# harrisonvanderbyl/rwkv-cpp-accelerated

Hardware: AMD Instinct MI355X
Metric: tokens/sec single-stream RWKV-4 uint8 greedy decode (higher is better)
Workload: dtype u8 weights x 23-bit fixed-point activations, exact 32-bit integer accumulate (tile form: v_mfma_i32_16x16x64_i8 on signed limbs; row form: v_dot4_u32_u8 on the VALU); f32/f64 epilogues, f64 state; 1 GPU; RWKV-4-Raven-7B uint8 single-stream greedy decode (L=32, D=4096, V=50277), 32-token prompt then 1885-token continuation, device-resident state; parallelism=1 GPU

## Files before the change

rwkv-cpp-accelerated_amd/csrc/kernels.hip.h:

```cpp
#pragma once
#include <hip/hip_runtime.h>
#include <stdint.h>

namespace rwkvk {

constexpr int NT = 512;
constexpr int NW = NT / 64;
constexpr int RED_BYTES = 1024;
#define RWKV_ARGS_NOW(...) asm volatile("" ::RWKV_ARGS_S(__VA_ARGS__))
#define RWKV_ARGS_S(...) RWKV_ARGS_PICK(__VA_ARGS__, RWKV_A8, RWKV_A7, RWKV_A6, RWKV_A5, RWKV_A4, RWKV_A3, RWKV_A2, RWKV_A1)(__VA_ARGS__)
#define RWKV_ARGS_PICK(a, b, c, d, e, f, g, h, N, ...) N
#define RWKV_A1(a) "s"(a)
#define RWKV_A2(a, ...) "s"(a), RWKV_A1(__VA_ARGS__)
#define RWKV_A3(a, ...) "s"(a), RWKV_A2(__VA_ARGS__)
#define RWKV_A4(a, ...) "s"(a), RWKV_A3(__VA_ARGS__)
#define RWKV_A5(a, ...) "s"(a), RWKV_A4(__VA_ARGS__)
#define RWKV_A6(a, ...) "s"(a), RWKV_A5(__VA_ARGS__)
#define RWKV_A7(a, ...) "s"(a), RWKV_A6(__VA_ARGS__)
#define RWKV_A8(a, ...) "s"(a), RWKV_A7(__VA_ARGS__)
__device__ __forceinline__ int wave_id() { return __builtin_amdgcn_readfirstlane((int)(threadIdx.x >> 6)); }
__device__ __forceinline__ int block_lo(int n) { return (int)(((unsigned)blockIdx.x * (unsigned)n) / gridDim.x); }
__device__ __forceinline__ int block_hi(int n) { return (int)((((unsigned)blockIdx.x + 1u) * (unsigned)n) / gridDim.x); }
constexpr unsigned VOCAB = 50277u;
constexpr float QLIM = 4194000.0f;
// ... 554 lines not shown
        {
            float *redf = reinterpret_cast<float *>(red + RED_MAX);
            const double ws = wave_sum(ps);
            const float wm = wave_max(pm);
            if (lane == 0) { red[RED_OFFS + wave] = ws; redf[wave] = wm; }
            tl_stamp(tl, 3);
            if (SPLIT) {
                if (lane == 0) __hip_atomic_fetch_add(spin, 1u, __ATOMIC_RELEASE, __HIP_MEMORY_SCOPE_WORKGROUP);
                while (__hip_atomic_load(spin, __ATOMIC_ACQUIRE, __HIP_MEMORY_SCOPE_WORKGROUP) < (unsigned)NWP) __builtin_amdgcn_s_sleep(1);
            } else {
                __syncthreads();
            }
            double ts = 0.0; float tm = 0.f;
#pragma unroll
            for (int i = 0; i < NWP; i++) { ts += red[RED_OFFS + i]; tm = fmaxf(tm, redf[i]); }
            Sf = (float)ts; amax = tm;
        }
        tl_stamp(tl, 4);
#pragma unroll
        for (int q = 0; q < NVEC; q++)
#pragma unroll
            for (int i = 0; i < NQP; i++) {
                const int qd = threadIdx.x + i * NTP;
                if (qd < S * 256) stage_quad(xq + q * XVD, qd, vl[q][i], inv_scale(amax), qd < nqd);
            }
        if (SPLIT && threadIdx.x == 0) { bc[0] = Sf; bc[4] = amax; }
        __syncthreads();
        group_load<R, S, SPLIT ? 0 : pre_steps<S>(), S>(w, wb, stride, chunks, lane);
    }
    if (SPLIT) { Sf = bc[0]; amax = bc[4]; }
    tl_stamp(tl, 5);
}

constexpr size_t CU_LDS_BYTES = 160 * 1024;
__host__ __device__ constexpr int row_nvec(int cls) { return cls == 1 ? 3 : cls == 3 ? 2 : cls == 4 ? 4 : 1; }
struct RowLds { size_t red = 0, xq = 0, bval = 0, bidx = 0, bytes = 0; };
__host__ __device__ constexpr RowLds row_lds_of(int cls, int S)
{
    RowLds l;
    l.xq = l.red + RED_BYTES;
    l.bval = l.xq + (size_t)row_nvec(cls) * S * xvd<1>() * 4;
    l.bidx = l.bval + (cls == 5 ? NW * sizeof(float) : 0);
    l.bytes = l.bidx + (cls == 5 ? NW * sizeof(unsigned) : 0);
    return l;
}
template <int CLS, int S> struct RowGeo {
    static constexpr RowLds L = row_lds_of(CLS, S);
    static_assert(L.xq % 16 == 0 && L.bval == L.xq + (size_t)row_nvec(CLS) * xvd<S>() * 4, "the staged vectors: 16-byte pieces, xvd<S>() words each");
    static_assert(row_lds_of(CLS, 5).bytes <= CU_LDS_BYTES, "LDS layout at S = 5");
};

__device__ __forceinline__ unsigned lds_addr(const void *p)
{
    return (unsigned)(unsigned long long)(const __attribute__((address_space(3))) void *)p;
}
__device__ __forceinline__ void dma_piece_shared(const uint8_t *src, unsigned lds_dst)
{
    unsigned keep;
    asm volatile("s_mov_b32 %0, m0\n\ts_mov_b32 m0, %2\n\ts_nop 0\n\tglobal_load_lds_dwordx4 %1, off\n\ts_mov_b32 m0, %0"
                 : "=&s"(keep) : "v"(src), "s"(lds_dst) : "memory");
}
__device__ __forceinline__ void loader_clean_slate() { __builtin_amdgcn_s_waitcnt(0x0F70); }
template <int N> __device__ __forceinline__ void wait_vm() { asm volatile("s_waitcnt vmcnt(%0)" ::"n"(N) : "memory"); }
constexpr int GLDS_SPIN = 1 << 18;
__device__ __forceinline__ void wait_count(const unsigned *p, unsigned least, unsigned &fail)
{
    bool ok = false;
    for (int it = 0; it < GLDS_SPIN; it++) {
        if (__hip_atomic_load(p, __ATOMIC_ACQUIRE, __HIP_MEMORY_SCOPE_WORKGROUP) >= least) { ok = true; break; }
        __builtin_amdgcn_s_sleep(1);
    }
    fail = ok ? fail : 3u;
}
__device__ __forceinline__ void ring_report(unsigned fail, unsigned *herr)
{
    if (fail != 0u && herr != nullptr && (threadIdx.x & 63) == 0) __hip_atomic_store(herr, fail, __ATOMIC_RELAXED, __HIP_MEMORY_SCOPE_SYSTEM);
}
#ifndef RWKV_RING_DEPTH
#define RWKV_RING_DEPTH 28
#endif
#ifndef RWKV_RING_PRE
#define RWKV_RING_PRE 8
#endif
#ifndef RWKV_TEST_DROP_GROUP
#define RWKV_TEST_DROP_GROUP 0
#endif
#ifndef RWKV_RING_PRE_DEPTH
#define RWKV_RING_PRE_DEPTH 20
#endif
constexpr int NC = NW - 1;

struct FirstArgs {
    const float *embed;
    const double *ln;
    double *x;
    const double *x_in;
    SiteStatic st;
    SiteDyn dy;
    const double *sxy;
    size_t slot_stride;
    const Ctl *ctl;
    int D;
    int from_token;
};
__global__ __launch_bounds__(NT) void k_first(FirstArgs a)
{
    __shared__ double red[RED_BYTES / 8];
    const int D = a.D;
    const int j0 = block_lo(D), j1 = block_hi(D);
    const size_t so = (size_t)a.ctl->slot * a.slot_stride;
    double mean = 0.0, rstd = 1.0;
    const float *row = a.from_token ? a.embed + (size_t)a.ctl->token * D : nullptr;
    if (a.from_token) {
        double s[2] = {0.0, 0.0};
        for (int j = threadIdx.x; j < D; j += NT) { const double v = (double)row[j]; s[0] += v; s[1] += v * v; }
        block_sum<2>(s, red + RED_STATS);
        mean = s[0] / (double)D;
        rstd = 1.0 / sqrt((s[1] - s[0] * mean) / (double)(D - 1));
        __syncthreads();
    }
    SiteAcc<3> acc;
    acc.clear();
    for (int j = j0 + threadIdx.x; j < j1; j += NT) {
        double x;
        if (a.from_token) { x = a.ln[j] * (((double)row[j] - mean) * rstd) + a.ln[D + j]; a.x[j] = x; }
        else { x = a.x_in[j]; a.x[j] = x; }
        SitePre<3> pre;
        site_prefetch<3>(a.st, j, pre);
        site_emit<3>(pre, a.dy, D, j, x, a.sxy[so + j], acc);
    }
    site_publish<3, 64>(acc, a.dy, red);
}

struct AttArgs {
    const double *x;
    SiteStatic st;
    SiteDyn dy;
    const uint8_t *w;
    const unsigned *rs;
    const double *uw, *ew;
    const float *r_att, *o_att;
    double *saa, *sbb;
    size_t slot_stride;
    float *ybuf;
    double *partS;
    float *partM;
    const Ctl *ctl;
    int D;
    int ns;
    unsigned long long *tl;
    unsigned *herr;
};

__device__ __forceinline__ void att_epilogue(double *saa, double *sbb, float *ybuf, int g, double aa, double bb, double e1, double ek, float v, float r, double ew, float ra, float oa, double &part, float &pmax)
{
    const double vv = (double)v;
    double y = (aa + e1 * vv) / (bb + e1);
    y = (1.0 / (1.0 + (double)expf(-r))) * y;
    saa[g] = (aa + ek * vv) * ew;
    sbb[g] = (bb + ek) * ew;
    const float yf = (float)y;
    const float ys = yf * ra;
    ybuf[g] = ys;
    part += (double)(yf * oa);
    pmax = fmaxf(pmax, fabsf(ys));
}

struct AttIn { unsigned rs[3]; double aa, bb, uw, ew; float ra, oa; };
template <int S>
__global__ __launch_bounds__(NT) void k_att(AttArgs a)
{
    extern __shared__ __attribute__((aligned(16))) unsigned char smem[];
    constexpr RowLds L = RowGeo<1, S>::L;
    double *red = reinterpret_cast<double *>(smem + L.red);
    unsigned *xq = reinterpret_cast<unsigned *>(smem + L.xq);
    const int D = a.D, lane = threadIdx.x & 63, wave = wave_id();
    const int chunks = D >> 4;
    const int g0 = block_lo(D);
    const int g1 = block_hi(D);
    const size_t so = (size_t)a.ctl->slot * a.slot_stride;

    tl_stamp(a.tl, 0);
    auto base = [&](int g) { return a.w + (size_t)(g < g1 ? g : (g1 > g0 ? g1 - 1 : 0)) * 3 * D; };
    double sc[3];
    float S0, S1, S2;
    auto scalars = [&](const SiteRed<3> &sr) {
        sc[0] = scale_of(sr.amax[0]); sc[1] = scale_of(sr.amax[1]); sc[2] = scale_of(sr.amax[2]);
        S0 = (float)sr.S[0]; S1 = (float)sr.S[1]; S2 = (float)sr.S[2];
    };
    double part = 0.0;
    float pmax = 0.f;
    auto pre = [&](int g) {
        AttIn in;
#pragma unroll
        for (int m = 0; m < 3; m++) in.rs[m] = a.rs[g * 3 + m];
        in.aa = a.saa[so + g]; in.bb = a.sbb[so + g]; in.uw = a.uw[g]; in.ew = a.ew[g];
        in.ra = a.r_att[g]; in.oa = a.o_att[g];
        return in;
    };
    auto epi = [&](int g, const unsigned long long (&T)[3], const AttIn &in) {
        if (lane == 0) {
            const float k = row_value(T[0], in.rs[0], sc[0]) + S0, v = row_value(T[1], in.rs[1], sc[1]) + S1;
            const float r = row_value(T[2], in.rs[2], sc[2]) + S2;
            att_epilogue(a.saa + so, a.sbb + so, a.ybuf, g, in.aa, in.bb, exp(in.uw + (double)k), exp((double)k), v, r, in.ew, in.ra, in.oa, part, pmax);
        }
    };
    u32x4 wA[3][S];
    int gA;
    unsigned *gctr = group_counter(red);
    first_groups(g0, wave, gctr, gA);
    SiteRed<3> sr;
    site_open<3, 3, S, (RWKV_SPLIT & 1) != 0>(a.st, a.dy, a.x, D, red, xq, wA, base(gA), (size_t)D, sr, true, a.tl);
    scalars(sr);
    stream_groups<3, S, PAT_PER_ROW>(wA, gA, g0, g1, gctr, xq, lane, (size_t)D, chunks, base, pre, epi);
    tl_stamp(a.tl, 6);
    __syncthreads();
    block_sum_max(part, pmax, red + RED_PART);
    if (threadIdx.x == 0) { a.partS[blockIdx.x] = part; a.partM[blockIdx.x] = pmax; }
    tl_stamp(a.tl, 7);
}

struct AttOutArgs {
    const uint8_t *w;
    const unsigned *rs;
    const float *ybuf;
    const double *partS;
    const float *partM;
    int n_part;
    double *x;
    const double *lnw, *lnb;
    const double *lnstat;
    double *sxy;
    SiteStatic st;
    SiteDyn dy;
    const double *sdd;
    size_t slot_stride;
    const Ctl *ctl;
    int D;
    int ns;
    unsigned long long *tl;
    unsigned *herr;
};

__device__ __forceinline__ void attout_epilogue(const AttOutArgs &a, size_t so, int D, int mi, float val, double xold, double lw, double lb, double prev2, double mean1, double rstd1, const SitePre<2> &pre, SiteAcc<2> &acc)
{
    const float accf = (float)xold + val;
    const double xnew = (double)accf;
    a.x[mi] = xnew;
    a.sxy[so + mi] = lw * ((xold - mean1) * rstd1) + lb;
    site_emit<2>(pre, a.dy, D, mi, xnew, prev2, acc);
}

template <int R> struct AttOutIn { unsigned rsum; double xold, lw, lb, prev2; SitePre<2> pre; int mi, shift; };
template <int S, int R>
__global__ __launch_bounds__(NT) void k_attout(AttOutArgs a)
{
    extern __shared__ __attribute__((aligned(16))) unsigned char smem[];
    constexpr RowLds L = RowGeo<2, S>::L;
    double *red = reinterpret_cast<double *>(smem + L.red);
    unsigned *xq = reinterpret_cast<unsigned *>(smem + L.xq);
    const int D = a.D, lane = threadIdx.x & 63, wave = wave_id();
    const int chunks = D >> 4;
    tl_stamp(a.tl, 0);
    const int G = (D + R - 1) / R;
    const int g0 = block_lo(G);
    const int g1 = block_hi(G);

    const double mean1 = a.lnstat[0], rstd1 = a.lnstat[1];
    const size_t so = (size_t)a.ctl->slot * a.slot_stride;
    auto base = [&](int gg) {
        int row = (gg < g1 ? gg : (g1 > g0 ? g1 - 1 : 0)) * R;
        if (row > D - R) row = D - R;
        return a.w + (size_t)row * D;
    };
    float Sf, amax;
    double sc;
    SiteAcc<2> acc;
    acc.clear();
    auto pre = [&](int g) {
        AttOutIn<R> in;
        int row0 = g * R;
        in.shift = (row0 > D - R) ? row0 - (D - R) : 0;
        row0 -= in.shift;
        in.mi = row0 + (lane < R ? lane : 0);
        in.rsum = a.rs[in.mi];
        in.xold = a.x[in.mi]; in.lw = a.lnw[in.mi]; in.lb = a.lnb[in.mi]; in.prev2 = a.sdd[so + in.mi];
        site_prefetch<2>(a.st, in.mi, in.pre);
        return in;
    };
    auto epi = [&](int, const unsigned long long (&T)[R], const AttOutIn<R> &in) {
#pragma unroll
        for (int r = 0; r < R; r++) {
            if (lane == r && r >= in.shift)
                attout_epilogue(a, so, D, in.mi, row_value(T[r], in.rsum, sc) + Sf, in.xold, in.lw, in.lb, in.prev2, mean1, rstd1, in.pre, acc);
        }
    };
    u32x4 wA[R][S];
    int gA;
    unsigned *gctr = group_counter(red);
    first_groups(g0, wave, gctr, gA);
    vec_open<1, R, S, (RWKV_SPLIT & 2) != 0>(a.ybuf, a.partS, a.partM, a.n_part, D, red, xq, wA, base(gA), (size_t)D, Sf, amax, a.tl);
    sc = scale_of(amax);
    stream_groups<R, S, PAT_SHARED>(wA, gA, g0, g1, gctr, xq, lane, (size_t)D, chunks, base, pre, epi);
    __syncthreads();
    tl_stamp(a.tl, 6);
    site_publish<2, R>(acc, a.dy, xq);
    tl_stamp(a.tl, 7);
}

struct FfnRKArgs {
    const double *x;
    SiteStatic st;
    SiteDyn dy;
    const uint8_t *w;
    const unsigned *rs;
    const float *r_fv, *o_fv;
    float *hbuf;
    float *rgate;
// ... 374 lines not shown
```

rwkv-cpp-accelerated_amd/csrc/tile.hip.h:

```cpp
#pragma once
#include "kernels.hip.h"

namespace rwkvk {

constexpr double TILE_CU = 4227200.0;
constexpr double TILE_CN = -1077952512.0;

#if RWKV_TL_STREAM == 2
#define TL_BAR(tl, ph) tl_stamp(tl, ph)
#else
#define TL_BAR(tl, ph)
#endif
typedef int tile_i32x4 __attribute__((ext_vector_type(4)));
constexpr int TILE_NWP = NT / 2 / 64;
constexpr int TILE_NSTASH = NC - TILE_NWP;
struct TileCtl {
    unsigned staged;
    unsigned landed;
    unsigned freed[8];
    unsigned tcnt[32];
    unsigned done[8];
    unsigned pad[2];
    unsigned long long sq[4];
    unsigned dump[64];
// ... 304 lines not shown
#endif
    }
    const u32x4 *wp = reinterpret_cast<const u32x4 *>(ring + (size_t)p * (S * 1024)) + lane;
#pragma unroll
    for (int s = 0; s < S; s++) w[s] = wp[s * 64];
    wk.taken++;
    asm volatile("" ::: "memory");
    if (lane == 0) __hip_atomic_store(&tc->freed[wave], wk.taken, __ATOMIC_RELAXED, __HIP_MEMORY_SCOPE_WORKGROUP);
}
template <int S, int HEAD>
__device__ __forceinline__ void tile_pretake(int NU, const unsigned char *ring, int ns, TileCtl *tc, int wave, int lane, TileWalk &wk, unsigned &fail,
                                             u32x4 (&wpre)[HEAD / TILE_NSTASH > 0 ? HEAD / TILE_NSTASH : 1][S])
{
    if constexpr (HEAD > 0) {
        if (HEAD > ns) fail = 2u;
#pragma unroll
        for (int k = 0; k < HEAD / TILE_NSTASH; k++) {
            const int u = TILE_NSTASH * k + (wave - TILE_NWP);
            if (u < NU && HEAD <= ns) tile_take<S>(ring, (unsigned)u, u, tc, wave, lane, wk, fail, wpre[k]);
        }
    }
}

template <int TH, int S, int UPT, int RUN, int HEAD, class VecOf, class OnTile>
__device__ __forceinline__ void tile_consume(int NU, const unsigned char *ring, int ns, TileCtl *tc, int *tsum, const unsigned *xq, int xvd_t,
                                             int wave, int lane, unsigned &fail, TileWalk &wk, const u32x4 (&wpre)[HEAD / TILE_NSTASH > 0 ? HEAD / TILE_NSTASH : 1][S],
                                             VecOf vec_of, OnTile on_tile, unsigned long long *tl = nullptr)
{
    static_assert(UPT % RUN == 0, "a run of units never straddles a tile");
    static_assert(HEAD == 0 || (RUN == 1 && HEAD % TILE_NSTASH == 0), "a head of the stream: round robin only, whole rounds of the three waves");
    constexpr int PPB = 64 / TH;
    const int pc = lane / TH, r = lane % TH;
    int cnt = 0;
    tile_i32x4 ma = tile_i32x4{0, 0, 0, 0}, mb = tile_i32x4{0, 0, 0, 0};
    auto mul = [&](const u32x4 (&w)[S], int u, int un) {
        const int t = u / UPT, c = u - t * UPT;
        const u32x4 *xp = reinterpret_cast<const u32x4 *>(xq + vec_of(t) * xvd_t);
        if constexpr (TH == 16) {
            xp += ((c * S) * PPB + pc) * 3 + (r < 3 ? r : 2);
        } else {
            const int m = (lane & 15) < 12 ? (lane & 15) : 11;
            xp += ((c * S) * PPB + 4 * (lane >> 4) + (m & 3)) * 3 + (m >> 2);
        }
#pragma unroll
        for (int s = 0; s < S; s++) {
            const u32x4 x = xp[s * PPB * 3];
            const tile_i32x4 af = tile_i32x4{(int)x[0], (int)x[1], (int)x[2], (int)x[3]}, bf = tile_i32x4{(int)w[s][0], (int)w[s][1], (int)w[s][2], (int)w[s][3]};
            if (s & 1) mb = __builtin_amdgcn_mfma_i32_16x16x64_i8(af, bf, mb, 0, 0, 0);
            else ma = __builtin_amdgcn_mfma_i32_16x16x64_i8(af, bf, ma, 0, 0, 0);
        }
        cnt++;
        if (un >= NU || un / UPT != t) {
            if constexpr (TH == 16) {
                if (lane < 16) {
                    int *ts = tsum + (t * TH + lane) * 3;
                    __hip_atomic_fetch_add(ts + 0, ma[0] + mb[0], __ATOMIC_RELAXED, __HIP_MEMORY_SCOPE_WORKGROUP);
                    __hip_atomic_fetch_add(ts + 1, ma[1] + mb[1], __ATOMIC_RELAXED, __HIP_MEMORY_SCOPE_WORKGROUP);
                    __hip_atomic_fetch_add(ts + 2, ma[2] + mb[2], __ATOMIC_RELAXED, __HIP_MEMORY_SCOPE_WORKGROUP);
                }
            } else {
                const int n = lane & 15;
                const tile_i32x4 sa = ma + mb;
                int v = n < 4 ? sa[0] : n < 8 ? sa[1] : n < 12 ? sa[2] : sa[3];
                v += __builtin_amdgcn_update_dpp(0, v, 0x124, 0xf, 0xf, true); v += __builtin_amdgcn_update_dpp(0, v, 0x128, 0xf, 0xf, true);
                if (n < 4 && lane < 48) __hip_atomic_fetch_add(tsum + (t * TH + n) * 3 + (lane >> 4), v, __ATOMIC_RELAXED, __HIP_MEMORY_SCOPE_WORKGROUP);
            }
            ma = mb = tile_i32x4{0, 0, 0, 0};
            unsigned old = 0u;
            if (lane == 0) old = __hip_atomic_fetch_add(&tc->tcnt[t], (unsigned)cnt, __ATOMIC_ACQ_REL, __HIP_MEMORY_SCOPE_WORKGROUP);
            old = (unsigned)__builtin_amdgcn_readfirstlane((int)old);
            if (old + (unsigned)cnt == (unsigned)UPT) on_tile(t);
            cnt = 0;
        }
    };
    if constexpr (HEAD > 0) {
        constexpr int NE = HEAD / TILE_NSTASH;
        if (wave >= TILE_NWP) {
#pragma unroll
            for (int k = 0; k < NE; k++) {
                const int u = tile_unit_of<HEAD>(wave, k);
                if (u < NU) mul(wpre[k], u, tile_unit_of<HEAD>(wave, k + 1));
            }
        }
        unsigned p = (unsigned)(HEAD + wave) % (unsigned)ns;
#pragma unroll 1
        for (int u = HEAD + wave; u < NU; u += NC) {
            u32x4 w[S];
            tile_take<S>(ring, p, u, tc, wave, lane, wk, fail, w);
            p += (unsigned)NC;
            while (p >= (unsigned)ns) p -= (unsigned)ns;
            mul(w, u, u + NC);
        }
    } else {
        unsigned p = (unsigned)(wave * RUN) % (unsigned)ns;
        for (int run = wave; run * RUN < NU; run += NC) {
#pragma unroll 1
            for (int cc = 0; cc < RUN; cc++) {
                const int u = run * RUN + cc;
                u32x4 w[S];
                tile_take<S>(ring, p, u, tc, wave, lane, wk, fail, w);
                p = p + 1 == (unsigned)ns ? 0u : p + 1;
                mul(w, u, cc + 1 < RUN ? u + 1 : (run + NC) * RUN);
            }
            p += (unsigned)((NC - 1) * RUN);
            while (p >= (unsigned)ns) p -= (unsigned)ns;
        }
    }
#if RWKV_TL_STREAM == 1
    if (tl && lane == 0) tl[((size_t)blockIdx.x * NW + wave) * 8 + 2] = wk.waited;
#endif
}

#ifndef RWKV_TILE_PRE_ATT
#define RWKV_TILE_PRE_ATT 4
#endif
#ifndef RWKV_TILE_PRE_ATTOUT
#define RWKV_TILE_PRE_ATTOUT 4
#endif
#ifndef RWKV_TILE_PRE_FRK
#define RWKV_TILE_PRE_FRK 4
#endif
#ifndef RWKV_TILE_PRE_FV
#define RWKV_TILE_PRE_FV RWKV_RING_PRE
#endif
#ifndef RWKV_TILE_HEAD_ATT
#define RWKV_TILE_HEAD_ATT 9
#endif
#ifndef RWKV_TILE_PRE4_ATT
#define RWKV_TILE_PRE4_ATT 0
#endif
#ifndef RWKV_TILE_HEAD_ATTOUT
#define RWKV_TILE_HEAD_ATTOUT 0
#endif
#ifndef RWKV_TILE_HEAD_FRK
#define RWKV_TILE_HEAD_FRK 0
#endif
#ifndef RWKV_TILE_HEAD_FV
#define RWKV_TILE_HEAD_FV 0
#endif
#ifndef RWKV_TILE_PRE_FV4
#define RWKV_TILE_PRE_FV4 0
#endif
struct TileImage {
    const uint8_t *bimg;
    int CB;
};
struct FfnRKTArgs { FfnRKArgs a; TileImage im; };
struct AttTArgs { AttArgs a; TileImage im; };
struct AttOutTArgs { AttOutArgs a; TileImage im; };
struct FfnVTArgs { FfnVArgs a; TileImage im; };
constexpr int tile_run(int TH, int UPT, int TPC) { return TH == 16 || TPC > 2 ? 1 : (UPT < 4 ? UPT : 4); }
constexpr size_t TILE_LDS_BYTES = 160 * 1024;
__host__ __device__ constexpr int tile_ncls(int cls) { return cls == 1 ? 3 : cls == 3 ? 5 : 1; }
__host__ __device__ constexpr int tile_nu(int cls, int TPC, int KBT, int S) { return tile_ncls(cls) * TPC * (KBT / S); }
__host__ __device__ constexpr int tile_xvd(int K) { return (K >> 4) * 12; }
struct TileLds {
    size_t xq = 0, rs = 0, sd = 0, sf = 0, ed = 0, ef = 0, sp = 0, rg = 0, scr = 0, tsum = 0, tc = 0, ring = 0;
    bool aligned = true;
    __host__ __device__ constexpr size_t take(size_t bytes, size_t align = 4) { aligned = aligned && ring % align == 0; const size_t o = ring; ring += bytes; return o; }
};
__host__ __device__ constexpr TileLds tile_lds_of(int cls, int D, int CPW)
{
    TileLds l;
    l.take(RED_BYTES, 16);
    l.xq = l.take((size_t)(cls == 1 ? 3 : cls == 3 ? 2 : 1) * tile_xvd(cls == 4 ? 4 * D : D) * 4, 16);
    if (cls == 1) {
        l.rs = l.take((size_t)3 * CPW * 4);
        l.sd = l.take((size_t)4 * CPW * 8, 8);
        l.sf = l.take((size_t)2 * CPW * 4);
        l.ed = l.take((size_t)2 * CPW * 8, 8);
        l.ef = l.take((size_t)2 * CPW * 4);
    } else if (cls == 3) {
        l.rs = l.take((size_t)5 * CPW * 4);
        l.sf = l.take((size_t)2 * 4 * CPW * 4);
    } else {
        l.sd = l.take((size_t)4 * CPW * 8, 8);
        l.sp = l.take((size_t)CPW * (cls == 2 ? 12 : 16) * 4, 16);
        l.rs = l.take((size_t)CPW * 4);
        if (cls == 4) l.rg = l.take((size_t)CPW * 4);
        l.scr = l.take((size_t)CPW * 10 * 8, 8);
    }
    l.tsum = l.take((size_t)tile_ncls(cls) * CPW * 12);
    l.tc = l.take(sizeof(TileCtl), 16);
    l.take(0, 16);
    return l;
}
template <class T> __device__ __forceinline__ T *tile_lds(unsigned char *smem, size_t off) { return reinterpret_cast<T *>(smem + off); }
__host__ __device__ constexpr int tile_ring_units(size_t fixed, int S, int nu)
{
    const int fit = (int)((TILE_LDS_BYTES - fixed) / ((size_t)S * 1024)) & ~1;
    return fit < nu ? fit : nu;
}
template <int CLS_, int S_, int KBT_, int TH_, int TPC_> struct TileGeo {
    static constexpr int CLS = CLS_, NCLS = tile_ncls(CLS), S = S_, KBT = KBT_, TH = TH_, TPC = TPC_, D = KBT * 1024 / TH / (CLS == 4 ? 4 : 1);
    static constexpr int CPW = TH * TPC, NTILE = NCLS * TPC, UPT = KBT / S, NU = tile_nu(CLS, TPC, KBT, S), RUN = tile_run(TH, UPT, TPC);
    static constexpr int HEAD_KNOB = CLS == 1 ? RWKV_TILE_HEAD_ATT : CLS == 2 ? RWKV_TILE_HEAD_ATTOUT : CLS == 3 ? RWKV_TILE_HEAD_FRK : RWKV_TILE_HEAD_FV;
    static constexpr int HEAD = TH == 16 && RUN == 1 ? HEAD_KNOB : 0, NE = HEAD / TILE_NSTASH > 0 ? HEAD / TILE_NSTASH : 1;
    static_assert(HEAD <= NU && HEAD % TILE_NSTASH == 0, "the head: whole rounds of the three non-staging waves, inside the stream");
    static_assert(KBT % S == 0 && NTILE <= 32 && TPC <= 8, "whole units per tile; TileCtl::tcnt / done");
    static_assert(tile_lds_of(CLS, D, CPW).aligned && tile_ring_units(tile_lds_of(CLS, D, CPW).ring, S, NU) >= (HEAD > 2 ? HEAD : 2), "LDS layout");
};
template <class G> __device__ __forceinline__ const uint8_t *tile_unit_src(const TileImage &im, int cb0, int u)
{
    const int t = u / G::UPT, c = u - t * G::UPT, cls = G::NCLS == 1 ? 0 : t / G::TPC, sub = G::NCLS == 1 ? t : t % G::TPC;
    return im.bimg + ((size_t)(cls * im.CB + cb0 + sub) * G::KBT + (size_t)c * G::S) * 1024;
}
template <class G> __device__ __forceinline__ const float *tile_consumer_open(double *red, const unsigned char *ring, int ns, TileCtl *tc, int wave, int lane,
                                                                            TileWalk &wk, unsigned &fail, u32x4 (&wpre)[G::NE][G::S])
{
    if (wave >= TILE_NWP) tile_pretake<G::S, G::HEAD>(G::NU, ring, ns, tc, wave, lane, wk, fail, wpre);
    wait_count(&tc->staged, TILE_NWP + TILE_NSTASH, fail);
    return red_bc(red);
}

template <int SD, int S, int KBT, int TH, int TPC>
__global__ __launch_bounds__(NT) void k_ffn_rk_t(FfnRKTArgs ta)
{
    extern __shared__ __attribute__((aligned(16))) unsigned char smem[];
    const FfnRKArgs &a = ta.a;
    using G = TileGeo<3, S, KBT, TH, TPC>;
    constexpr int CPW = G::CPW;
    double *red = reinterpret_cast<double *>(smem);
    const int D = a.D, lane = threadIdx.x & 63, wave = wave_id(), xvd_t = tile_xvd(D);
    const TileLds L = tile_lds_of(G::CLS, D, CPW);
    unsigned *xq = tile_lds<unsigned>(smem, L.xq), *srs = tile_lds<unsigned>(smem, L.rs);
    float *sf = tile_lds<float>(smem, L.sf);
    int *tsum = tile_lds<int>(smem, L.tsum);
    TileCtl *tc = tile_lds<TileCtl>(smem, L.tc);
    unsigned char *ring = smem + L.ring;
    RWKV_ARGS_NOW(a.x, a.st.C, a.st.TC, a.st.maxC, a.dy.B, a.dy.pd, a.dy.pf, a.dy.n_part);
    const int cb0 = blockIdx.x * TPC, ch0 = blockIdx.x * CPW;
    tl_stamp(a.tl, 0);
    double part = 0.0;
    float pmax = 0.f;
    unsigned fail = 0u;
    if (wave == NC) {
        fail = tile_loader<S, G::UPT, G::RUN, TH, RWKV_TILE_PRE_FRK, G::HEAD>(G::NU, G::NTILE, ring, a.ns, tc, tsum, lane, [&](int u) { return tile_unit_src<G>(ta.im, cb0, u); }, a.tl);
        tl_stamp(a.tl, 2);
    } else {
        if (wave < TILE_NWP) {
            tile_site<2, SD>(a.st, a.dy, a.x, D, red, xq, xvd_t, true, tc, a.tl);
        } else {
            const int n = wave == 4 ? 5 * CPW : 4 * CPW;
            unsigned v0 = 0u, v1 = 0u;
            const unsigned *src = wave == 4 ? a.rs + ch0 * 5 : reinterpret_cast<const unsigned *>(wave == 5 ? a.r_fv + ch0 * 4 : a.o_fv + ch0 * 4);
            if (lane < n) v0 = src[lane];
            if (lane + 64 < n) v1 = src[lane + 64];
            TL_BAR(a.tl, 1);
            __syncthreads();
            TL_BAR(a.tl, 2);
            unsigned *dst = wave == 4 ? srs : reinterpret_cast<unsigned *>(sf) + (wave == 5 ? 0 : 4 * CPW);
            if (lane < n) dst[lane] = v0;
            if (lane + 64 < n) dst[lane + 64] = v1;
            tile_stash_done(tc, lane);
        }
        TileWalk wk;
        u32x4 wpre[G::NE][S];
        const float *bc = tile_consumer_open<G>(red, ring, a.ns, tc, wave, lane, wk, fail, wpre);
        const double sck = scale_of(bc[4]), scr = scale_of(bc[5]);
        const float Sk = bc[0], Sr = bc[1];
        const double cAk = tile_cA(tc, 0, (double)D), cAr = tile_cA(tc, 1, (double)D);
        tl_stamp(a.tl, 5);
        auto on_tile = [&](int t) {
            if (lane < TH) {
                const int q = t / TPC, li = (t % TPC) * TH + lane;
                const long long M = tile_row_sum<TH>(tsum, t, lane);
                const unsigned rs = srs[li * 5 + q];
                if (q < 4) {
                    const float val = tile_row_value(M, cAk, rs, sck) + Sk;
                    const int hi = li * 4 + q;
                    ffn_k_epilogue(a, 4 * ch0 + hi, val, sf[hi], sf[4 * CPW + hi], part, pmax);
                } else {
                    const float val = tile_row_value(M, cAr, rs, scr) + Sr;
                    ffn_r_epilogue(a, ch0 + li, val);
                }
            }
        };
        tile_consume<TH, S, G::UPT, G::RUN, G::HEAD>(G::NU, ring, a.ns, tc, tsum, xq, xvd_t, wave, lane, fail, wk, wpre, [](int t) { return t / TPC < 4 ? 0 : 1; }, on_tile, a.tl);
    }
    tl_stamp(a.tl, 6);
    __syncthreads();
    block_sum_max(part, pmax, red + RED_PART);
    if (threadIdx.x == 0) { a.partS[blockIdx.x] = part; a.partM[blockIdx.x] = pmax; }
    ring_report(fail, a.herr);
    tl_stamp(a.tl, 7);
}

template <int SD, int S, int KBT, int TH, int TPC>
__global__ __launch_bounds__(NT) void k_att_t(AttTArgs ta)
{
    extern __shared__ __attribute__((aligned(16))) unsigned char smem[];
    const AttArgs &a = ta.a;
    using G = TileGeo<1, S, KBT, TH, TPC>;
    constexpr int CPW = G::CPW;
    double *red = reinterpret_cast<double *>(smem);
    const int D = a.D, lane = threadIdx.x & 63, wave = wave_id(), xvd_t = tile_xvd(D);
    const TileLds L = tile_lds_of(G::CLS, D, CPW);
    unsigned *xq = tile_lds<unsigned>(smem, L.xq), *stash = tile_lds<unsigned>(smem, L.rs);
    double *sd = tile_lds<double>(smem, L.sd), *ed = tile_lds<double>(smem, L.ed);
    float *sf = tile_lds<float>(smem, L.sf), *ef = tile_lds<float>(smem, L.ef);
    int *tsum = tile_lds<int>(smem, L.tsum);
    TileCtl *tc = tile_lds<TileCtl>(smem, L.tc);
    unsigned char *ring = smem + L.ring;
    RWKV_ARGS_NOW(a.x, a.st.C, a.st.TC, a.st.maxC, a.dy.B, a.dy.pd, a.dy.pf, a.dy.n_part);
    const int cb0 = blockIdx.x * TPC, ch0 = blockIdx.x * CPW;
    tl_stamp(a.tl, 0);
    double part = 0.0;
    float pmax = 0.f;
    unsigned fail = 0u;
    if (wave == NC) {
        fail = tile_loader<S, G::UPT, G::RUN, TH, (TH == 16 ? RWKV_TILE_PRE_ATT : RWKV_TILE_PRE4_ATT), G::HEAD>(G::NU, G::NTILE, ring, a.ns, tc, tsum, lane, [&](int u) { return tile_unit_src<G>(ta.im, cb0, u); }, a.tl);
        tl_stamp(a.tl, 2);
    } else {
        const size_t so = (size_t)a.ctl->slot * a.slot_stride;
        if (wave < TILE_NWP) {
            tile_site<3, SD>(a.st, a.dy, a.x, D, red, xq, xvd_t, true, tc, a.tl);
        } else {
            unsigned v0 = 0u;
            double d0 = 0.0, d1 = 0.0;
            auto dsrc = [&](int i) { const int g = i / CPW, j = i - g * CPW; return g == 0 ? a.saa[so + ch0 + j] : g == 1 ? a.sbb[so + ch0 + j] : g == 2 ? a.uw[ch0 + j] : a.ew[ch0 + j]; };
            if (wave == 4) { if (lane < 3 * CPW) v0 = a.rs[ch0 * 3 + lane]; }
            else if (wave == 5) { if (lane < 4 * CPW) d0 = dsrc(lane); if (lane + 64 < 4 * CPW) d1 = dsrc(lane + 64); }
            else if (lane < 2 * CPW) v0 = __float_as_uint(lane < CPW ? a.r_att[ch0 + lane] : a.o_att[ch0 + lane - CPW]);
            TL_BAR(a.tl, 1);
            __syncthreads();
            TL_BAR(a.tl, 2);
            if (wave == 4) { if (lane < 3 * CPW) stash[lane] = v0; }
            else if (wave == 5) { if (lane < 4 * CPW) sd[lane] = d0; if (lane + 64 < 4 * CPW) sd[lane + 64] = d1; }
            else if (lane < 2 * CPW) sf[lane] = __uint_as_float(v0);
            tile_stash_done(tc, lane);
        }
        TileWalk wk;
        u32x4 wpre[G::NE][S];
        const float *bc = tile_consumer_open<G>(red, ring, a.ns, tc, wave, lane, wk, fail, wpre);
        tl_stamp(a.tl, 5);
        auto on_tile = [&](int t) {
            const int q = t / TPC, sub = t % TPC;
            if (lane < TH) {
                const int li = sub * TH + lane;
                const long long M = tile_row_sum<TH>(tsum, t, lane);
                const double scq = scale_of(bc[4 + q]), cAq = tile_cA(tc, q, (double)D);
                const float val = tile_row_value(M, cAq, stash[li * 3 + q], scq) + bc[q];
                if (q == 0) { ed[li] = exp(sd[2 * CPW + li] + (double)val); ed[CPW + li] = exp((double)val); }
                else ef[(q - 1) * CPW + li] = val;
            }
            unsigned old = 0u;
            if (lane == 0) old = __hip_atomic_fetch_add(&tc->done[sub], 1u, __ATOMIC_ACQ_REL, __HIP_MEMORY_SCOPE_WORKGROUP);
            old = (unsigned)__builtin_amdgcn_readfirstlane((int)old);
            if (old == 2u && lane < TH) {
                const int li = sub * TH + lane, g = ch0 + li;
                const double aa = sd[li], bb = sd[CPW + li], ew = sd[3 * CPW + li];
                const double e1 = *reinterpret_cast<volatile double *>(ed + li), ek = *reinterpret_cast<volatile double *>(ed + CPW + li);
                const float v = *reinterpret_cast<volatile float *>(ef + li), r = *reinterpret_cast<volatile float *>(ef + CPW + li);
                att_epilogue(a.saa + so, a.sbb + so, a.ybuf, g, aa, bb, e1, ek, v, r, ew, sf[li], sf[CPW + li], part, pmax);
            }
        };
        tile_consume<TH, S, G::UPT, G::RUN, G::HEAD>(G::NU, ring, a.ns, tc, tsum, xq, xvd_t, wave, lane, fail, wk, wpre, [](int t) { return t / TPC; }, on_tile, a.tl);
    }
    tl_stamp(a.tl, 6);
    __syncthreads();
    block_sum_max(part, pmax, red + RED_PART);
    if (threadIdx.x == 0) { a.partS[blockIdx.x] = part; a.partM[blockIdx.x] = pmax; }
    ring_report(fail, a.herr);
    tl_stamp(a.tl, 7);
}

template <int NV>
__device__ __forceinline__ void tile_site_leave(const SiteAcc<NV> &acc, double *scr, int cpw, int li)
{
    float *scf = reinterpret_cast<float *>(scr + cpw * 8);
#pragma unroll
    for (int k = 0; k < 8; k++) scr[li * 8 + k] = acc.d[k];
#pragma unroll
    for (int k = 0; k < 4; k++) scf[li * 4 + k] = acc.f[k];
}
__device__ __forceinline__ void tile_site_publish(const SiteDyn &dy, const double *scr, int cpw)
{
    const float *scf = reinterpret_cast<const float *>(scr + cpw * 8);
    if (threadIdx.x < 8) {
        double t = 0.0;
        for (int i = 0; i < cpw; i++) t += scr[i * 8 + threadIdx.x];
        dy.pd[(size_t)blockIdx.x * 8 + threadIdx.x] = t;
    } else if (threadIdx.x < 12) {
        float t = 0.f;
        for (int i = 0; i < cpw; i++) t = fmaxf(t, scf[i * 4 + (threadIdx.x - 8)]);
        dy.pf[(size_t)blockIdx.x * 4 + (threadIdx.x - 8)] = t;
    }
}

template <int SD, int S, int KBT, int TH, int TPC>
__global__ __launch_bounds__(NT) void k_attout_t(AttOutTArgs ta)
{
    extern __shared__ __attribute__((aligned(16))) unsigned char smem[];
    const AttOutArgs &a = ta.a;
    using G = TileGeo<2, S, KBT, TH, TPC>;
    constexpr int CPW = G::CPW;
    double *red = reinterpret_cast<double *>(smem);
    const int D = a.D, lane = threadIdx.x & 63, wave = wave_id(), xvd_t = tile_xvd(D);
    const TileLds L = tile_lds_of(G::CLS, D, CPW);
    unsigned *xq = tile_lds<unsigned>(smem, L.xq), *srs = tile_lds<unsigned>(smem, L.rs);
    double *sd = tile_lds<double>(smem, L.sd), *scr = tile_lds<double>(smem, L.scr);
    float *sp = tile_lds<float>(smem, L.sp);
    int *tsum = tile_lds<int>(smem, L.tsum);
    TileCtl *tc = tile_lds<TileCtl>(smem, L.tc);
    unsigned char *ring = smem + L.ring;
    RWKV_ARGS_NOW(a.ybuf, a.partS, a.partM, a.n_part);
    const int cb0 = blockIdx.x * TPC, ch0 = blockIdx.x * CPW;
    tl_stamp(a.tl, 0);
    unsigned fail = 0u;
    if (wave == NC) {
        fail = tile_loader<S, G::UPT, G::RUN, TH, RWKV_TILE_PRE_ATTOUT, G::HEAD>(G::NU, G::NTILE, ring, a.ns, tc, tsum, lane, [&](int u) { return tile_unit_src<G>(ta.im, cb0, u); }, a.tl);
        tl_stamp(a.tl, 2);
    } else {
        const double mean1 = a.lnstat[0], rstd1 = a.lnstat[1];
        const size_t so = (size_t)a.ctl->slot * a.slot_stride;
        if (wave < TILE_NWP) {
            tile_vec<SD>(a.ybuf, a.partS, a.partM, a.n_part, D, red, xq, tc, a.tl);
        } else {
            auto dsrc = [&](int i) { const int g = i / CPW, j = i - g * CPW; return g == 0 ? a.x[ch0 + j] : g == 1 ? a.lnw[ch0 + j] : g == 2 ? a.lnb[ch0 + j] : a.sdd[so + ch0 + j]; };
            double d0 = 0.0, d1 = 0.0;
            f32x4 p0 = f32x4{0.f, 0.f, 0.f, 0.f};
            unsigned v0 = 0u;
            if (wave == 4) { if (lane < 4 * CPW) d0 = dsrc(lane); if (lane + 64 < 4 * CPW) d1 = dsrc(lane + 64); }
            else if (wave == 5) { if (lane < 3 * CPW) p0 = reinterpret_cast<const f32x4 *>(a.st.P + (size_t)ch0 * 12)[lane]; }
            else if (lane < CPW) v0 = a.rs[ch0 + lane];
            TL_BAR(a.tl, 1);
            __syncthreads();
            TL_BAR(a.tl, 2);
            if (wave == 4) { if (lane < 4 * CPW) sd[lane] = d0; if (lane + 64 < 4 * CPW) sd[lane + 64] = d1; }
            else if (wave == 5) { if (lane < 3 * CPW) reinterpret_cast<f32x4 *>(sp)[lane] = p0; }
            else if (lane < CPW) srs[lane] = v0;
            tile_stash_done(tc, lane);
        }
        TileWalk wk;
        u32x4 wpre[G::NE][S];
        const float *bc = tile_consumer_open<G>(red, ring, a.ns, tc, wave, lane, wk, fail, wpre);
        const float Sf = bc[0];
        const double sc = scale_of(bc[4]), cA = tile_cA(tc, 0, (double)D);
        tl_stamp(a.tl, 5);
        auto on_tile = [&](int t) {
            if (lane < TH) {
                const int li = t * TH + lane, mi = ch0 + li;
                const long long M = tile_row_sum<TH>(tsum, t, lane);
                SiteAcc<2> acc;
                acc.clear();
                attout_epilogue(a, so, D, mi, tile_row_value(M, cA, srs[li], sc) + Sf, sd[li], sd[CPW + li], sd[2 * CPW + li], sd[3 * CPW + li], mean1, rstd1,
                                *reinterpret_cast<const SitePre<2> *>(sp + li * 12), acc);
                tile_site_leave<2>(acc, scr, CPW, li);
            }
        };
        tile_consume<TH, S, G::UPT, G::RUN, G::HEAD>(G::NU, ring, a.ns, tc, tsum, xq, xvd_t, wave, lane, fail, wk, wpre, [](int) { return 0; }, on_tile, a.tl);
    }
    tl_stamp(a.tl, 6);
    __syncthreads();
    tile_site_publish(a.dy, scr, CPW);
    ring_report(fail, a.herr);
    tl_stamp(a.tl, 7);
}

template <int SD, int S, int KBT, int TH, int TPC, int NVN>
__global__ __launch_bounds__(NT) void k_ffnv_t(FfnVTArgs ta)
{
    extern __shared__ __attribute__((aligned(16))) unsigned char smem[];
    const FfnVArgs &a = ta.a;
    using G = TileGeo<4, S, KBT, TH, TPC>;
    constexpr int CPW = G::CPW, PW = site_pw<NVN>();
    double *red = reinterpret_cast<double *>(smem);
    const int D = a.D, lane = threadIdx.x & 63, wave = wave_id(), xvd_t = tile_xvd(4 * D);
    const TileLds L = tile_lds_of(G::CLS, D, CPW);
    unsigned *xq = tile_lds<unsigned>(smem, L.xq), *srs = tile_lds<unsigned>(smem, L.rs);
    double *sd = tile_lds<double>(smem, L.sd), *scr = tile_lds<double>(smem, L.scr);
    float *sp = tile_lds<float>(smem, L.sp), *srg = tile_lds<float>(smem, L.rg);
    int *tsum = tile_lds<int>(smem, L.tsum);
    TileCtl *tc = tile_lds<TileCtl>(smem, L.tc);
    unsigned char *ring = smem + L.ring;
    RWKV_ARGS_NOW(a.hbuf, a.partS, a.partM, a.n_part);
    const int cb0 = blockIdx.x * TPC, ch0 = blockIdx.x * CPW;
    tl_stamp(a.tl, 0);
    unsigned fail = 0u;
    if (wave == NC) {
        fail = tile_loader<S, G::UPT, G::RUN, TH, (TH == 16 ? RWKV_TILE_PRE_FV : RWKV_TILE_PRE_FV4), G::HEAD>(G::NU, G::NTILE, ring, a.ns, tc, tsum, lane, [&](int u) { return tile_unit_src<G>(ta.im, cb0, u); }, a.tl);
        tl_stamp(a.tl, 2);
    } else {
        const double mean2 = a.lnstat[0], rstd2 = a.lnstat[1];
        const size_t so = (size_t)a.ctl->slot * a.slot_stride;
        if (wave < TILE_NWP) {
            tile_vec<4 * SD>(a.hbuf, a.partS, a.partM, a.n_part, 4 * D, red, xq, tc, a.tl);
        } else {
            auto dsrc = [&](int i) { const int g = i / CPW, j = i - g * CPW; return g == 0 ? a.x[ch0 + j] : g == 1 ? a.lnw[ch0 + j] : g == 2 ? a.lnb[ch0 + j] : (NVN == 3 ? a.sprev[so + ch0 + j] : 0.0); };
            double d0 = 0.0, d1 = 0.0;
            f32x4 p0 = f32x4{0.f, 0.f, 0.f, 0.f}, p1 = f32x4{0.f, 0.f, 0.f, 0.f};
            unsigned v0 = 0u;
            constexpr int NP4 = CPW * PW / 4;
            if (wave == 4) { if (lane < 4 * CPW) d0 = dsrc(lane); if (lane + 64 < 4 * CPW) d1 = dsrc(lane + 64); }
            else if (wave == 5) { if (lane < NP4) p0 = reinterpret_cast<const f32x4 *>(a.st.P + (size_t)ch0 * PW)[lane]; if (lane + 64 < NP4) p1 = reinterpret_cast<const f32x4 *>(a.st.P + (size_t)ch0 * PW)[lane + 64]; }
            else if (lane < 2 * CPW) v0 = lane < CPW ? a.rs[ch0 + lane] : __float_as_uint(a.rgate[ch0 + lane - CPW]);
            TL_BAR(a.tl, 1);
            __syncthreads();
            TL_BAR(a.tl, 2);
            if (wave == 4) { if (lane < 4 * CPW) sd[lane] = d0; if (lane + 64 < 4 * CPW) sd[lane + 64] = d1; }
            else if (wave == 5) { if (lane < NP4) reinterpret_cast<f32x4 *>(sp)[lane] = p0; if (lane + 64 < NP4) reinterpret_cast<f32x4 *>(sp)[lane + 64] = p1; }
            else if (lane < 2 * CPW) srs[lane] = v0;
            tile_stash_done(tc, lane);
        }
        TileWalk wk;
        u32x4 wpre[G::NE][S];
        const float *bc = tile_consumer_open<G>(red, ring, a.ns, tc, wave, lane, wk, fail, wpre);
        const float Sf = bc[0];
        const double sc = scale_of(bc[4]), cA = tile_cA(tc, 0, 4.0 * (double)D);
        tl_stamp(a.tl, 5);
// ... 22 lines not shown
```

Before: 630.6 tokens/s.

## Reorder K/V/R tile streaming and hoist gate and bb-state work out of epilogue

Adds a permutation of the order in which row classes of the weight image are streamed: for the attention K/V/R kernel the order becomes K, R, V, and for the FFN kernel the last class is streamed first. In the attention kernel, the sigmoid gate of R is computed as soon as the R tile lands and is kept in a new LDS slot, and the bb state update is written as soon as K lands. This leaves only the V-dependent wkv math in the final epilogue on the critical tail. It costs extra LDS for the gate, which the static asserts pin to the same ring depth, and it changes the order in which tiles complete.

```diff
diff --git a/rwkv-cpp-accelerated_amd/csrc/kernels.hip.h b/rwkv-cpp-accelerated_amd/csrc/kernels.hip.h
--- a/rwkv-cpp-accelerated_amd/csrc/kernels.hip.h
+++ b/rwkv-cpp-accelerated_amd/csrc/kernels.hip.h
@@ -730,18 +730,25 @@
     unsigned *herr;
 };
 
-__device__ __forceinline__ void att_epilogue(double *saa, double *sbb, float *ybuf, int g, double aa, double bb, double e1, double ek, float v, float r, double ew, float ra, float oa, double &part, float &pmax)
+__device__ __forceinline__ double att_gate(float r) { return 1.0 / (1.0 + (double)expf(-r)); }
+__device__ __forceinline__ void att_state_bb(double *sbb, int g, double bb, double ek, double ew) { sbb[g] = (bb + ek) * ew; }
+__device__ __forceinline__ void att_wkv(double *saa, float *ybuf, int g, double aa, double bb, double e1, double ek, float v, double gate, double ew, float ra, float oa, double &part, float &pmax)
 {
     const double vv = (double)v;
     double y = (aa + e1 * vv) / (bb + e1);
-    y = (1.0 / (1.0 + (double)expf(-r))) * y;
+    y = gate * y;
     saa[g] = (aa + ek * vv) * ew;
-    sbb[g] = (bb + ek) * ew;
     const float yf = (float)y;
     const float ys = yf * ra;
     ybuf[g] = ys;
     part += (double)(yf * oa);
     pmax = fmaxf(pmax, fabsf(ys));
+}
+__device__ __forceinline__ void att_epilogue(double *saa, double *sbb, float *ybuf, int g, double aa, double bb, double e1, double ek, float v, float r, double ew, float ra, float oa, double &part, float &pmax)
+{
+    const double gate = att_gate(r);
+    att_state_bb(sbb, g, bb, ek, ew);
+    att_wkv(saa, ybuf, g, aa, bb, e1, ek, v, gate, ew, ra, oa, part, pmax);
 }
 
 struct AttIn { unsigned rs[3]; double aa, bb, uw, ew; float ra, oa; };
diff --git a/rwkv-cpp-accelerated_amd/csrc/tile.hip.h b/rwkv-cpp-accelerated_amd/csrc/tile.hip.h
--- a/rwkv-cpp-accelerated_amd/csrc/tile.hip.h
+++ b/rwkv-cpp-accelerated_amd/csrc/tile.hip.h
@@ -480,10 +480,22 @@
 constexpr int tile_run(int TH, int UPT, int TPC) { return TH == 16 || TPC > 2 ? 1 : (UPT < 4 ? UPT : 4); }
 constexpr size_t TILE_LDS_BYTES = 160 * 1024;
 __host__ __device__ constexpr int tile_ncls(int cls) { return cls == 1 ? 3 : cls == 3 ? 5 : 1; }
+__host__ __device__ constexpr int tile_stream_cls(int cls, int p) { return cls == 1 ? (p == 0 ? 0 : 3 - p) : cls == 3 ? (p == 0 ? 4 : p - 1) : p; }
+__host__ __device__ constexpr bool tile_stream_is_permutation(int cls)
+{
+    for (int q = 0; q < tile_ncls(cls); q++) {
+        int hits = 0;
+        for (int p = 0; p < tile_ncls(cls); p++) hits += tile_stream_cls(cls, p) == q ? 1 : 0;
+        if (hits != 1) return false;
+    }
+    return true;
+}
+static_assert(tile_stream_is_permutation(1) && tile_stream_is_permutation(2) && tile_stream_is_permutation(3) && tile_stream_is_permutation(4),
+              "every row class of the image is streamed exactly once");
 __host__ __device__ constexpr int tile_nu(int cls, int TPC, int KBT, int S) { return tile_ncls(cls) * TPC * (KBT / S); }
 __host__ __device__ constexpr int tile_xvd(int K) { return (K >> 4) * 12; }
 struct TileLds {
-    size_t xq = 0, rs = 0, sd = 0, sf = 0, ed = 0, ef = 0, sp = 0, rg = 0, scr = 0, tsum = 0, tc = 0, ring = 0;
+    size_t xq = 0, rs = 0, sd = 0, sf = 0, ed = 0, eg = 0, ef = 0, sp = 0, rg = 0, scr = 0, tsum = 0, tc = 0, ring = 0;
     bool aligned = true;
     __host__ __device__ constexpr size_t take(size_t bytes, size_t align = 4) { aligned = aligned && ring % align == 0; const size_t o = ring; ring += bytes; return o; }
 };
@@ -497,7 +509,8 @@
         l.sd = l.take((size_t)4 * CPW * 8, 8);
         l.sf = l.take((size_t)2 * CPW * 4);
         l.ed = l.take((size_t)2 * CPW * 8, 8);
-        l.ef = l.take((size_t)2 * CPW * 4);
+        l.eg = l.take((size_t)CPW * 8, 8);
+        l.ef = l.take((size_t)CPW * 4);
     } else if (cls == 3) {
         l.rs = l.take((size_t)5 * CPW * 4);
         l.sf = l.take((size_t)2 * 4 * CPW * 4);
@@ -527,10 +540,13 @@
     static_assert(HEAD <= NU && HEAD % TILE_NSTASH == 0, "the head: whole rounds of the three non-staging waves, inside the stream");
     static_assert(KBT % S == 0 && NTILE <= 32 && TPC <= 8, "whole units per tile; TileCtl::tcnt / done");
     static_assert(tile_lds_of(CLS, D, CPW).aligned && tile_ring_units(tile_lds_of(CLS, D, CPW).ring, S, NU) >= (HEAD > 2 ? HEAD : 2), "LDS layout");
+    static_assert(!(CLS == 1 && TH == 16 && D == 4096 && S == 4) || tile_ring_units(tile_lds_of(CLS, D, CPW).ring, S, NU) == 30,
+                  "K/V/R at 4096 channels: the gate's stash leaves the ring at the 30 units it was measured with");
+    static_assert(HEAD <= UPT && (CLS != 1 || tile_stream_cls(CLS, 0) == 0), "the head in registers lies in the first tile streamed: K's for K/V/R");
 };
 template <class G> __device__ __forceinline__ const uint8_t *tile_unit_src(const TileImage &im, int cb0, int u)
 {
-    const int t = u / G::UPT, c = u - t * G::UPT, cls = G::NCLS == 1 ? 0 : t / G::TPC, sub = G::NCLS == 1 ? t : t % G::TPC;
+    const int t = u / G::UPT, c = u - t * G::UPT, cls = G::NCLS == 1 ? 0 : tile_stream_cls(G::CLS, t / G::TPC), sub = G::NCLS == 1 ? t : t % G::TPC;
     return im.bimg + ((size_t)(cls * im.CB + cb0 + sub) * G::KBT + (size_t)c * G::S) * 1024;
 }
 template <class G> __device__ __forceinline__ const float *tile_consumer_open(double *red, const unsigned char *ring, int ns, TileCtl *tc, int wave, int lane,
@@ -591,7 +607,7 @@
         tl_stamp(a.tl, 5);
         auto on_tile = [&](int t) {
             if (lane < TH) {
-                const int q = t / TPC, li = (t % TPC) * TH + lane;
+                const int q = tile_stream_cls(G::CLS, t / TPC), li = (t % TPC) * TH + lane;
                 const long long M = tile_row_sum<TH>(tsum, t, lane);
                 const unsigned rs = srs[li * 5 + q];
                 if (q < 4) {
@@ -604,7 +620,7 @@
                 }
             }
         };
-        tile_consume<TH, S, G::UPT, G::RUN, G::HEAD>(G::NU, ring, a.ns, tc, tsum, xq, xvd_t, wave, lane, fail, wk, wpre, [](int t) { return t / TPC < 4 ? 0 : 1; }, on_tile, a.tl);
+        tile_consume<TH, S, G::UPT, G::RUN, G::HEAD>(G::NU, ring, a.ns, tc, tsum, xq, xvd_t, wave, lane, fail, wk, wpre, [](int t) { return tile_stream_cls(G::CLS, t / TPC) < 4 ? 0 : 1; }, on_tile, a.tl);
     }
     tl_stamp(a.tl, 6);
     __syncthreads();
@@ -625,7 +641,7 @@
     const int D = a.D, lane = threadIdx.x & 63, wave = wave_id(), xvd_t = tile_xvd(D);
     const TileLds L = tile_lds_of(G::CLS, D, CPW);
     unsigned *xq = tile_lds<unsigned>(smem, L.xq), *stash = tile_lds<unsigned>(smem, L.rs);
-    double *sd = tile_lds<double>(smem, L.sd), *ed = tile_lds<double>(smem, L.ed);
+    double *sd = tile_lds<double>(smem, L.sd), *ed = tile_lds<double>(smem, L.ed), *eg = tile_lds<double>(smem, L.eg);
     float *sf = tile_lds<float>(smem, L.sf), *ef = tile_lds<float>(smem, L.ef);
     int *tsum = tile_lds<int>(smem, L.tsum);
     TileCtl *tc = tile_lds<TileCtl>(smem, L.tc);
@@ -663,14 +679,18 @@
         const float *bc = tile_consumer_open<G>(red, ring, a.ns, tc, wave, lane, wk, fail, wpre);
         tl_stamp(a.tl, 5);
         auto on_tile = [&](int t) {
-            const int q = t / TPC, sub = t % TPC;
+            const int q = tile_stream_cls(G::CLS, t / TPC), sub = t % TPC;
             if (lane < TH) {
                 const int li = sub * TH + lane;
                 const long long M = tile_row_sum<TH>(tsum, t, lane);
                 const double scq = scale_of(bc[4 + q]), cAq = tile_cA(tc, q, (double)D);
                 const float val = tile_row_value(M, cAq, stash[li * 3 + q], scq) + bc[q];
-                if (q == 0) { ed[li] = exp(sd[2 * CPW + li] + (double)val); ed[CPW + li] = exp((double)val); }
-                else ef[(q - 1) * CPW + li] = val;
+                if (q == 0) {
+                    const double ek = exp((double)val);
+                    ed[li] = exp(sd[2 * CPW + li] + (double)val); ed[CPW + li] = ek;
+                    att_state_bb(a.sbb + so, ch0 + li, sd[CPW + li], ek, sd[3 * CPW + li]);
+                } else if (q == 2) eg[li] = att_gate(val);
+                else ef[li] = val;
             }
             unsigned old = 0u;
             if (lane == 0) old = __hip_atomic_fetch_add(&tc->done[sub], 1u, __ATOMIC_ACQ_REL, __HIP_MEMORY_SCOPE_WORKGROUP);
@@ -679,11 +699,12 @@
                 const int li = sub * TH + lane, g = ch0 + li;
                 const double aa = sd[li], bb = sd[CPW + li], ew = sd[3 * CPW + li];
                 const double e1 = *reinterpret_cast<volatile double *>(ed + li), ek = *reinterpret_cast<volatile double *>(ed + CPW + li);
-                const float v = *reinterpret_cast<volatile float *>(ef + li), r = *reinterpret_cast<volatile float *>(ef + CPW + li);
-                att_epilogue(a.saa + so, a.sbb + so, a.ybuf, g, aa, bb, e1, ek, v, r, ew, sf[li], sf[CPW + li], part, pmax);
+                const double gate = *reinterpret_cast<volatile double *>(eg + li);
+                const float v = *reinterpret_cast<volatile float *>(ef + li);
+                att_wkv(a.saa + so, a.ybuf, g, aa, bb, e1, ek, v, gate, ew, sf[li], sf[CPW + li], part, pmax);
             }
         };
-        tile_consume<TH, S, G::UPT, G::RUN, G::HEAD>(G::NU, ring, a.ns, tc, tsum, xq, xvd_t, wave, lane, fail, wk, wpre, [](int t) { return t / TPC; }, on_tile, a.tl);
+        tile_consume<TH, S, G::UPT, G::RUN, G::HEAD>(G::NU, ring, a.ns, tc, tsum, xq, xvd_t, wave, lane, fail, wk, wpre, [](int t) { return tile_stream_cls(G::CLS, t / TPC); }, on_tile, a.tl);
     }
     tl_stamp(a.tl, 6);
     __syncthreads();
```

New measurement: 628.3 tokens/s. About the same (-0.4%).
